# kepingbi/ProdSearch

Measured on AMD Instinct MI355X. Metric: train (u,q,i,neg) tuples/sec at bs=384, 20 neg, d=128, higher is better.
Workload: dtype f32 (fp32 MFMA and VALU; wide products, the fused per-replica kernels and grouped weight gradients as fp32-grade bf16x3 products: exact 3-way bf16 split of both fp32 operands, 6 of the 9 cross products as bf16 MFMAs per step, fp32 accumulation); 1 GPU; item_transformer d=128 1 layer 8 heads ff=512 uprev=20 bs=384/GPU 20 neg Q=8 W=1 P=18357 V=32387 dropout=0.10 (BASELINE configs[1]); global_batch=384, parallelism=dp1, step=sample+fwd+bwd+clip/Adam via nn.Module API (trainer.py:74-78), replicas_per_row=21

## Files before the change

### prodsearch_amd/csrc/rowwise.h

```cpp
#pragma once
#include "common.h"

struct ScoreArgs {
  int B, K, W, C, R, d;
  FDiv fK1, fWK1, fC;
  int64_t P, V;
  int bias_product, pos_weight;
  const int64_t* target; const int64_t* neg_items; const int64_t* pos_words; const int64_t* neg_words;
  const int64_t* candi;
  const float* product_emb; const float* word_emb; const float* product_bias; const float* word_bias;
  const float* enc;
  float* item_scores;
  float* word_scores;
  float* loss_parts;
  float* item_terms;
  float* word_terms;
  float* loss3;
  float* loss_acc;
  float* loss_blk;
  int loss_nblk;
  float scale;
  const float* scale_dev;
  float* denc;
  int part;
  int items_elsewhere;
  float* g_product_emb; float* g_word_emb; float* g_product_bias; float* g_word_bias;
  float* word_blk; int word_nblk; float* item_blk; uint32_t* ticket;
  const float* samp_prob; const int32_t* samp_alias; uint32_t samp_step, samp_k0, samp_k1; int samp_inline;
  unsigned long long* stamp;
};
#define PS_WORD_TASKS_PER_WG 16
inline void score_finish(ScoreArgs& a) {
  a.fK1 = make_fdiv(a.K + 1); a.fWK1 = make_fdiv(a.W * (a.K + 1)); a.fC = make_fdiv(a.C > 0 ? a.C : 1);
}
int launch_score_fwd(ScoreArgs& a, hipStream_t st);
int launch_loss(const ScoreArgs& a, hipStream_t st);
int launch_score_bwd(const ScoreArgs& a, hipStream_t st);

struct WSplit {
  const float* w[3]; int rows[3], cols[3];
  uint16_t* fwd_wo; uint16_t* fwd_ff; uint16_t* bwd_ff; uint16_t* bwd_wo;
  int on;
  const float* wkv[2]; uint16_t* fwd_kv;
  uint16_t* bwd_kv;
};
__host__ __device__ inline int wsplit_chunks(const WSplit& W, int ) {
  const int d = W.cols[0], F = W.rows[1];
  return (d * d + 2 * d * F) / 8 + (W.wkv[0] ? 2 * d * d / 8 : 0);
}
#if defined(__HIPCC__)
__device__ inline void wsplit_chunk(const WSplit& W, int set, int q) {
  const int d = W.cols[0], F = W.rows[1];
  const int n_wo = d * d / 8, n_ff = 2 * d * F / 8, n_kv = W.wkv[0] ? 2 * d * d / 8 : 0;
  if (q >= n_wo + n_ff + n_kv) return;
  uint16_t* dst;
  int which;
  if (q < n_wo) { which = set ? 3 : 0; dst = set ? W.bwd_wo : W.fwd_wo; }
  else if (q < n_wo + n_ff) { which = set ? 2 : 1; q -= n_wo; dst = set ? W.bwd_ff : W.fwd_ff; }
  else { which = set ? 5 : 4; q -= n_wo + n_ff; dst = set ? W.bwd_kv : W.fwd_kv; }
  const int step = q >> 6, ln = q & 63, l31 = ln & 31, hh = ln >> 5;
  const int phi = 16 * ((l31 >> 2) & 1) + 4 * (l31 >> 3) + (l31 & 3);
  const float* src; int stride;
  if (which == 0) { const int nb = step >> 3, t = step & 7; src = W.w[0] + (size_t)(32 * nb + phi) * d + 16 * t + 8 * hh; stride = 1; }
  else if (which == 4) { const int nb = step >> 3, t = step & 7; src = W.wkv[nb >> 2] + (size_t)(32 * (nb & 3) + phi) * d + 16 * t + 8 * hh; stride = 1; }
  else if (which == 5) {
    const int hg = step >> 5, nb = (step >> 3) & 3, t = step & 7;
    src = W.wkv[t >> 2] + (size_t)(64 * hg + 16 * (t & 3) + 8 * hh) * d + 32 * nb + phi; stride = d;
  }
  else if (which == 3) { const int kb = step >> 3, t = step & 7; src = W.w[0] + (size_t)(16 * t + 8 * hh) * d + 32 * kb + phi; stride = d; }
  else {
    const int fb = step >> 4, r = step & 15;
    if (r < 8) {
      if (which == 1) { src = W.w[1] + (size_t)(32 * fb + phi) * d + 16 * r + 8 * hh; stride = 1; }
      else { src = W.w[2] + (size_t)(16 * r + 8 * hh) * F + 32 * fb + phi; stride = F; }
    } else {
      const int t = (r - 8) >> 2, nb = (r - 8) & 3, kf = 32 * fb + 16 * hh + 8 * t;
      if (which == 1) { src = W.w[2] + (size_t)(32 * nb + phi) * F + kf; stride = 1; }
      else { src = W.w[1] + (size_t)kf * d + 32 * nb + phi; stride = d; }
    }
  }
  float x[8];
  if (stride == 1) {
    const float4 v0 = *reinterpret_cast<const float4*>(src), v1 = *reinterpret_cast<const float4*>(src + 4);
    x[0] = v0.x; x[1] = v0.y; x[2] = v0.z; x[3] = v0.w; x[4] = v1.x; x[5] = v1.y; x[6] = v1.z; x[7] = v1.w;
  } else {
#pragma unroll
    for (int e = 0; e < 8; ++e) x[e] = src[(size_t)e * stride];
  }
  uint32_t wd[3][4];
#pragma unroll
  for (int i = 0; i < 4; ++i) {
    uint16_t hb[2][3];
#pragma unroll
    for (int e = 0; e < 2; ++e) {
      const float xv = x[2 * i + e];
      const __bf16 bh = (__bf16)xv;
      float r = xv - (float)bh;
      const __bf16 bm = (__bf16)r;
      r -= (float)bm;
      const __bf16 bl = (__bf16)r;
      hb[e][0] = __builtin_bit_cast(uint16_t, bh); hb[e][1] = __builtin_bit_cast(uint16_t, bm); hb[e][2] = __builtin_bit_cast(uint16_t, bl);
    }
#pragma unroll
    for (int pl = 0; pl < 3; ++pl) wd[pl][i] = (uint32_t)hb[0][pl] | ((uint32_t)hb[1][pl] << 16);
  }
#pragma unroll
  for (int pl = 0; pl < 3; ++pl)
    *reinterpret_cast<uint4*>(dst + ((size_t)(step * 3 + pl) * 64 + ln) * 8) = make_uint4(wd[pl][0], wd[pl][1], wd[pl][2], wd[pl][3]);
}
#endif
struct EmbedArgs {
  int B, Q, L, S, d;
  int64_t P, V;
  int tem;
  int fs;
  const float* fs_w; const float* fs_b;
  int32_t* vrows; int32_t* vcount;
  int samp_wgs;
  int use_pos;
  const int64_t* qw; const int64_t* ui;
  const float* word_emb; const float* hist_tab; const float* pe;
  DropSpec drop_fs;
  float* qmean_d;
  float* query_emb;
  float* x;
  const float* samp_prob; const int32_t* samp_alias; int64_t* samp_items; int64_t* samp_words;
  int samp_nitem, samp_nword; uint32_t samp_step, samp_k0, samp_k1;
  int fold_words; ScoreArgs sc; int word_wgs, list_wgs;
  WSplit split; int split_wgs;
  int split_fwd_only;
  uint32_t* clear_word;
  int32_t* zero_i32; int zero_n, zero_wgs;
};
int launch_embed_fwd(const EmbedArgs& a, hipStream_t st);

struct LnFwdArgs {
  const float* x; int ldx; float* y; int ldy; float* stats;
  const float* g; const float* b; int rows, d; float eps;
};
int launch_ln_fwd(const LnFwdArgs& a, hipStream_t st);

struct LnBwdArgs {
  const float* dy; int lddy;
  const float* x; int ldx;
  const float* stats; const float* g;
  int rows, d;
  ResMap res;
  float* dx; int lddx;
  float* out2;
  DropSpec drop2;
  float* colsum;
  float* dgamma; float* dbeta;
  float* partial;
};
int launch_ln_bwd(const LnBwdArgs& a, hipStream_t st);
int ln_bwd_blocks(int rows);

#define PS_MAX_COLFOLD 8
struct ColFold { const float* partial; int nblk, d; float* dst[3]; };
struct ColFoldList { ColFold e[PS_MAX_COLFOLD]; int n; };

struct AttnArgs {
  int n_in, fan, H, S, Sq, d, dh, qpos;
  FDiv fS, fd, fdh, fd4, fHS, fHQS;
  int jc;
  int seq_div;
  int L; int64_t P; const int64_t* ui;
  const float* valid;
  const float* kp; const float* vp; const float* qp;
  float* attn;
  float* ctx;
  DropSpec drop;
  const float* dctx;
  float* dq; int lddq;
  float* dkv; int lddkv;
  float* dbq; float* dbk; float* dbv;
  float* bias_part;
  float qscale;
  const float* wq; float* dxq_part;
  const float* fanin_src;
  uint32_t* sig; uint32_t sigval;
  const uint16_t* kvb_stream; float* dxp[2];
};
inline void attn_finish(AttnArgs& a) {
  a.fS = make_fdiv(a.S); a.fd = make_fdiv(a.d); a.fdh = make_fdiv(a.dh); a.fd4 = make_fdiv(a.d / 4);
  a.fHS = make_fdiv(a.H * a.S); a.fHQS = make_fdiv((a.H / 4 > 0 ? a.H / 4 : 1) * a.S);
}
int launch_attn_fwd(const AttnArgs& a, hipStream_t st);
int launch_attn_bwd(const AttnArgs& a, hipStream_t st);
struct KvqArgs {
  AttnArgs at;
  const float* x;
  const uint16_t* kv_stream;
  const float* bk; const float* bv; const float* wq; const float* bq;
  float* kp; float* vp; float* qp;
  uint32_t* amask;
  unsigned long long* stamp;
  WSplit split;
};
bool kvq_attn_fits(const AttnArgs& a);
int launch_kvq_attn_fwd(const KvqArgs& a, hipStream_t st);
int launch_attn_fwd_sq1(const AttnArgs& a, hipStream_t st);
int launch_attn_bwd_sq1(const AttnArgs& a, hipStream_t st);
bool attn_sq1_fits(const AttnArgs& a);
bool attn_w1_fits(const AttnArgs& a);
int launch_attn_bwd_w1(const AttnArgs& a, bool pads_unread, hipStream_t st);
int launch_attn_fwd_w1(const AttnArgs& a, hipStream_t st);
bool attn_wf_fits(const AttnArgs& a);
int launch_attn_fwd_wf(const AttnArgs& a, uint32_t* amask, hipStream_t st);
int launch_attn_bwd_wf(const AttnArgs& a, const uint32_t* amask, bool pads_unread, hipStream_t st, bool* key_split = nullptr);
bool attn_bwd_wf_two_partials(const AttnArgs& a);
int attn_sq1_split(const AttnArgs& a);

struct EmbedBwdArgs {
  int B, Q, L, S, d;
  int64_t P, V;
  int tem;
  const int64_t* qw; const int64_t* ui;
  const float* dx;
  const float* dx2;
  const float* dqmean_d;
  DropSpec drop_fs;
  float* g_hist_tab; float* g_word_emb;
  const float* fw_dy; const float* fw_x; float* g_fs_w;
  const float* fsb_dqe; int fsb_lddqe; const float* fsb_qe; const float* fsb_w; float* g_fs_b;
  const float* fsb_dqe2; float fsb_k2;
  float* fsb_dqpre_out;
  ColFoldList fold;
  float* det_dm;
  uint32_t* sig; uint32_t sigval;
};
int launch_embed_scatter(const EmbedBwdArgs& a, hipStream_t st);
int launch_rows_scatter_det(const int32_t* keys, int ntask, const float* src, int64_t ld, int d, float* table, hipStream_t st,
                            const float* scale = nullptr, const int32_t* rowidx = nullptr);

int launch_fanin_sum(const float* src, int ld, int n_in, int fan, int d, float* out, hipStream_t st);
int launch_tanh_bwd(const float* dqe, int lddqe, const float* qe, float* dqpre, float* dfb, int rows, int d,
                    hipStream_t st);

struct StageArgs {
  const int64_t* src[6]; int64_t* dst[6]; int n[6];
  uint32_t step; uint32_t* step_word;
  const float* prob; const int32_t* alias;
  int nitem, nword; int64_t P, V; uint32_t k0, k1;
};
int launch_stage(const StageArgs& a, hipStream_t st);
const void* stage_kernel_handle();
const void* loss_kernel_handle();
int score_fwd_blocks(const ScoreArgs& a);

int launch_sample(const PsTemDesc& d, const float* alias_prob, const int32_t* alias_idx, int64_t* neg_items,
                  int64_t* neg_words, hipStream_t st);

struct MlpFwdArgs {
  int M, F;
  int fan, S, qpos;
  const float* ctx; const float* xin;
  const float *wo, *bo, *g1, *be1, *w1, *b1, *w2, *b2, *gf, *bef;
  DropSpec drop_ctx, drop_ff1, drop_ff2;
  float *y1, *ln1, *st1, *a1, *h1, *y2, *stf, *enc;
  int fold_score; ScoreArgs sc;
  WSplit x3;
  unsigned long long* stamp;
};
int launch_mlp_fwd_fused(const MlpFwdArgs& a, hipStream_t st);
bool mlp_fwd_can_fold_score(int M, int F, int d);
bool mlp_x3_enabled(int F);
bool mlp_fused_serves(int d, int F);
int64_t mlp_x3_floats(int d, int F);
bool ps_fusion_enabled();

struct MlpBwdArgs {
  int M, F;
  const float* denc;
  const float* item_scores; const int64_t* target; const int64_t* neg_items; const float* product_emb;
  int B, K, pos_weight; int64_t P; float scale; const float* scale_dev;
  const float* enc; float* g_product_emb; float* g_product_bias;
  const float* y2; const float* stf; const float* gf;
  const float* y1; const float* st1; const float* g1;
  const float* a1;
  const float *wo, *w1, *w2;
  DropSpec drop_ctx, drop_ff1, drop_ff2;
  float* do2;
  float* da1;
  float* dy1;
  float* dout;
  float* dctx;
  float* part_f;
  float* part_1;
  float* part_b1;
  WSplit x3;
  uint32_t* sig; uint32_t sigval;
  unsigned long long* stamp;
};
int launch_mlp_bwd_fused(const MlpBwdArgs& a, hipStream_t st);
int mlp_bwd_fused_blocks(int M);
int mlp_bwd_b1_rows(int M, int F);
```

### prodsearch_amd/csrc/rowwise.hip

```cpp
#include "rowwise.h"
#include "side_stream.h"
#include <stdlib.h>

static inline int lpr_for(int d) {
  int n = d / 4, l = 1;
  while (l < n && l < 64) l <<= 1;
  return l;
}

__device__ inline int64_t clamp_idx(int64_t i, int64_t hi) { return i < 0 ? hi : (i > hi ? hi : i); }

struct Task {
  const float* row; const float* vec; float bias; float* out;
  float* term; float tw;
  float lw;
};
__device__ inline Task score_task(const ScoreArgs& a, int t) {
  Task k;
  const int K1 = a.K + 1;
  if (a.C > 0) {
    int b = fdiv(t, a.fC);
    int64_t idx = clamp_idx(a.candi[t], a.P);
    k.row = a.product_emb + (size_t)idx * a.d;
    k.vec = a.enc + (size_t)b * a.R * a.d;
    k.bias = a.bias_product ? a.product_bias[idx] : 0.f;
    k.out = a.item_scores + t;
    k.term = nullptr; k.tw = 0.f; k.lw = 0.f;
    return k;
  }
  const int nitem = a.B * K1;
  if (t < nitem) {
    int b = fdiv(t, a.fK1), j = t - b * K1;
    int64_t idx = clamp_idx(j == 0 ? a.target[b] : a.neg_items[(size_t)b * a.K + j - 1], a.P);
    k.row = a.product_emb + (size_t)idx * a.d;
    k.vec = a.enc + ((size_t)b * a.R + (a.R > 1 ? j : 0)) * a.d;
    k.bias = a.bias_product ? a.product_bias[idx] : 0.f;
    k.out = a.item_scores + t;
    k.term = a.item_terms + t;
    k.tw = j == 0 ? -(a.pos_weight ? (float)a.K : 1.f) : 1.f;
    k.lw = 1.f;
  } else {
    int u = t - nitem;
    int b = fdiv(u, a.fWK1), r = u - b * (a.W * K1);
    int w = fdiv(r, a.fK1), j = r - w * K1;
    int64_t widx;
    if (j == 0) widx = a.pos_words[(size_t)b * a.W + w];
    else if (a.samp_inline) {
      const uint32_t su = (uint32_t)(b * a.W * a.K + w * a.K + j - 1);
      Philox4 rr = philox4x32_10(su, 0u, PS_SITE_SAMPLE_WORD, a.samp_step, a.samp_k0, a.samp_k1);
      const int64_t i = (int64_t)(((uint64_t)rr.x * (uint64_t)a.V) >> 32);
      const float f = (float)(rr.y >> 8) * (1.0f / 16777216.0f);
      widx = f < a.samp_prob[i] ? i : (int64_t)a.samp_alias[i];
    } else widx = a.neg_words[(size_t)b * a.W * a.K + (size_t)w * a.K + j - 1];
    int64_t idx = clamp_idx(widx, a.V - 1);
    int64_t tb = clamp_idx(a.target[b], a.P);
    k.row = a.word_emb + (size_t)idx * a.d;
    k.vec = a.product_emb + (size_t)tb * a.d;
    k.bias = a.word_bias[idx];
    k.out = a.word_scores + u;
    k.term = a.word_terms + u;
    k.tw = j == 0 ? -1.f : 1.f;
    int cnt = 0;
    for (int ww = 0; ww < a.W; ++ww) cnt += a.pos_words[(size_t)b * a.W + ww] != a.V - 1;
    const bool valid = a.pos_words[(size_t)b * a.W + w] != a.V - 1;
    k.lw = valid ? -1.f / (float)cnt : -0.f;
  }
  return k;
}


__device__ inline void word_tasks_wg(const ScoreArgs& a, int wg) {
  __shared__ float wred[16];
  const int tid = threadIdx.x, grp = tid >> 4, c = tid & 15;
  const int nitem = a.B * (a.K + 1), nword = a.B * a.W * (a.K + 1);
  const int nch = a.d >> 2;
  float cil = 0.f;
  if (wg == 0 && tid < 18) a.ticket[tid] = 0u;
  for (int pass = 0; pass < PS_WORD_TASKS_PER_WG / 16; ++pass) {
    const int u = wg * PS_WORD_TASKS_PER_WG + pass * 16 + grp;
    float s = 0.f;
    Task k;
    k.out = nullptr;
    if (u < nword) {
      k = score_task(a, nitem + u);
      for (int cc = c; cc < nch; cc += 16) {
        const float4 r = *reinterpret_cast<const float4*>(k.row + 4 * cc);
        const float4 v = *reinterpret_cast<const float4*>(k.vec + 4 * cc);
        s += r.x * v.x + r.y * v.y + r.z * v.z + r.w * v.w;
      }
    }
    s = group_sum(s, 16);
    if (c == 0 && k.out) {
      const float sc = s + k.bias;
      *k.out = sc;
      const float term = fabsf(k.tw) * softplus_f(k.tw < 0.f ? -sc : sc);
      *k.term = term;
      cil -= term * k.lw;
    }
  }
  if (c == 0) wred[grp] = cil;
  __syncthreads();
  if (tid == 0) {
    float q = 0.f;
    for (int g2 = 0; g2 < 16; ++g2) q += wred[g2];
    a.word_blk[wg] = q;
  }
}

__global__ __launch_bounds__(256) void embed_fwd_kernel(const EmbedArgs a) {
  extern __shared__ float red[];
  if ((int)blockIdx.x >= a.B && (int)blockIdx.x < a.B + a.samp_wgs) {
    const int t = ((int)blockIdx.x - a.B) * 256 + (int)threadIdx.x;
    if (t < a.samp_nitem) {
      Philox4 r = philox4x32_10((uint32_t)t, 0u, PS_SITE_SAMPLE_ITEM, a.samp_step, a.samp_k0, a.samp_k1);
      a.samp_items[t] = (int64_t)(((uint64_t)r.x * (uint64_t)a.P) >> 32);
    } else if (t < a.samp_nitem + a.samp_nword) {
      const int u = t - a.samp_nitem;
      Philox4 r = philox4x32_10((uint32_t)u, 0u, PS_SITE_SAMPLE_WORD, a.samp_step, a.samp_k0, a.samp_k1);
      const int64_t i = (int64_t)(((uint64_t)r.x * (uint64_t)a.V) >> 32);
      const float f = (float)(r.y >> 8) * (1.0f / 16777216.0f);
      a.samp_words[u] = f < a.samp_prob[i] ? i : (int64_t)a.samp_alias[i];
    }
    return;
  }
  if ((int)blockIdx.x >= a.B + a.samp_wgs + a.list_wgs + a.word_wgs + a.split_wgs) {
    const int i = (((int)blockIdx.x - a.B - a.samp_wgs - a.list_wgs - a.word_wgs - a.split_wgs) * 256 + (int)threadIdx.x) * 4;
    if (i + 3 < a.zero_n) *reinterpret_cast<int4*>(a.zero_i32 + i) = make_int4(0, 0, 0, 0);
    else for (int j = i; j < a.zero_n; ++j) a.zero_i32[j] = 0;
    return;
  }
  if ((int)blockIdx.x >= a.B + a.samp_wgs + a.list_wgs + a.word_wgs) {
    const int q = ((int)blockIdx.x - a.B - a.samp_wgs - a.list_wgs - a.word_wgs) * 256 + (int)threadIdx.x;
    const int n0 = wsplit_chunks(a.split, 0);
    if (q < n0) wsplit_chunk(a.split, 0, q);
    else if (!a.split_fwd_only) wsplit_chunk(a.split, 1, q - n0);
    return;
  }
  if ((int)blockIdx.x >= a.B + a.samp_wgs + a.list_wgs) {
    word_tasks_wg(a.sc, (int)blockIdx.x - a.B - a.samp_wgs - a.list_wgs);
    return;
  }
  if ((int)blockIdx.x >= a.B + a.samp_wgs) {
    __shared__ int vred[4];
    const int b = (int)blockIdx.x - a.B - a.samp_wgs, tid = threadIdx.x;
    int cntp = 0;
    {
      const int n = b * a.L;
      const bool al16 = (reinterpret_cast<uintptr_t>(a.ui) & 15) == 0;
      if (al16) {
        const longlong2* u2 = reinterpret_cast<const longlong2*>(a.ui);
        const int n2 = n >> 1;
        for (int i = tid; i < n2; i += 4 * 256) {
          longlong2 v[4];
#pragma unroll
          for (int u = 0; u < 4; ++u) { const int j = i + 256 * u; v[u] = u2[j < n2 ? j : 0]; }
#pragma unroll
          for (int u = 0; u < 4; ++u) {
            const int j = i + 256 * u;
            cntp += (j < n2 && v[u].x != a.P) + (j < n2 && v[u].y != a.P);
          }
        }
        if ((n & 1) && tid == 0) cntp += (a.ui[n - 1] != a.P);
      } else {
        for (int i = tid; i < n; i += 256) cntp += (a.ui[i] != a.P);
      }
    }
    const bool mine = tid < a.L && a.ui[(size_t)b * a.L + tid] != a.P;
    const unsigned long long vm = __ballot(mine);
    cntp = (int)wave_sum((float)cntp);
    if ((tid & 63) == 0) vred[tid >> 6] = cntp;
    __syncthreads();
    const int off = vred[0] + vred[1] + vred[2] + vred[3] + b;
    if (tid == 0) a.vrows[off] = b * a.S;
    if (mine) a.vrows[off + 1 + __popcll(vm & ((1ull << tid) - 1ull))] = b * a.S + 1 + tid;
    if (tid == 0 && b == a.B - 1) *a.vcount = off + 1 + __popcll(vm);
    return;
  }
  const int b = blockIdx.x, tid = threadIdx.x;
  if (b == 0 && tid == 0 && a.clear_word) { a.clear_word[0] = 0u; a.clear_word[1] = 0u; a.clear_word[2] = 0u; a.clear_word[3] = 0u; }
  const int d = a.d, nchunk = d >> 2;
  const int rpp = 256 / nchunk;
  const int rg = tid / nchunk, c = tid - rg * nchunk;
  const bool active = rg < rpp;
  const bool fuse_fs = a.fs && a.fs_w;
  float* mean_s = red + (size_t)rpp * d;
  const bool fs_pre = fuse_fs && d == 128;
  float4 wpre[16];
  float4 bpre = make_float4(0.f, 0.f, 0.f, 0.f);
  if (fs_pre) {
#pragma unroll
    for (int u = 0; u < 16; ++u) wpre[u] = *reinterpret_cast<const float4*>(a.fs_w + (size_t)(rg + 8 * u) * 128 + 4 * c);
  }
  if (fuse_fs && tid < nchunk) bpre = *reinterpret_cast<const float4*>(a.fs_b + 4 * c);
  const int64_t wpad = a.V - 1;
  int cnt = 0;
  for (int q = 0; q < a.Q; ++q) cnt += (a.qw[(size_t)b * a.Q + q] != wpad);
  float4 acc = make_float4(0.f, 0.f, 0.f, 0.f);
  if (active) {
    for (int q = rg; q < a.Q; q += rpp) {
      int64_t idx = a.qw[(size_t)b * a.Q + q];
      if (idx != wpad && idx >= 0 && idx < a.V) {
        float4 v = *reinterpret_cast<const float4*>(a.word_emb + (size_t)idx * d + 4 * c);
        acc.x += v.x; acc.y += v.y; acc.z += v.z; acc.w += v.w;
      }
    }
    *reinterpret_cast<float4*>(red + (size_t)rg * d + 4 * c) = acc;
  }
  __syncthreads();
  if (tid < nchunk) {
    float4 s = make_float4(0.f, 0.f, 0.f, 0.f);
    for (int r = 0; r < rpp; ++r) {
      float4 v = *reinterpret_cast<const float4*>(red + (size_t)r * d + 4 * c);
      s.x += v.x; s.y += v.y; s.z += v.z; s.w += v.w;
    }
    const float inv = 1.f / (float)(cnt > 0 ? cnt : 1);
    float m[4] = {s.x * inv, s.y * inv, s.z * inv, s.w * inv};
#pragma unroll
    for (int e = 0; e < 4; ++e) m[e] *= drop_mult(a.drop_fs, (uint32_t)b, (uint32_t)(4 * c + e));
    float4 md = make_float4(m[0], m[1], m[2], m[3]);
    *reinterpret_cast<float4*>(a.qmean_d + (size_t)b * d + 4 * c) = md;
    if (fuse_fs) *reinterpret_cast<float4*>(mean_s + 4 * c) = md;
    if (!a.fs) {
      *reinterpret_cast<float4*>(a.query_emb + (size_t)b * d + 4 * c) = md;
      if (a.tem) {
        float4 o = md;
        if (a.use_pos) {
          float4 p = *reinterpret_cast<const float4*>(a.pe + 4 * c);
          o.x += p.x; o.y += p.y; o.z += p.z; o.w += p.w;
        }
        *reinterpret_cast<float4*>(a.x + (size_t)b * a.S * d + 4 * c) = o;
      }
    }
  }
  if (a.tem && active) {
    for (int l = rg; l < a.L; l += rpp) {
      int64_t idx = a.ui[(size_t)b * a.L + l];
      float4 v = make_float4(0.f, 0.f, 0.f, 0.f);
      if (idx != a.P && idx >= 0 && idx < a.P)
        v = *reinterpret_cast<const float4*>(a.hist_tab + (size_t)idx * d + 4 * c);
      if (a.use_pos) {
        float4 p = *reinterpret_cast<const float4*>(a.pe + (size_t)(1 + l) * d + 4 * c);
        v.x += p.x; v.y += p.y; v.z += p.z; v.w += p.w;
      }
      *reinterpret_cast<float4*>(a.x + ((size_t)b * a.S + 1 + l) * d + 4 * c) = v;
    }
  }
  if (!fuse_fs) return;
  __syncthreads();
  float* out_s = mean_s + d;
  if (fs_pre) {
    const float4 mv = *reinterpret_cast<const float4*>(mean_s + 4 * c);
#pragma unroll
    for (int u = 0; u < 16; ++u) {
      const float4 wv = wpre[u];
      const float s = half_sum_last(wv.x * mv.x + wv.y * mv.y + wv.z * mv.z + wv.w * mv.w);
      if (c == 31) out_s[rg + 8 * u] = s;
    }
  } else {
    int lpr = 1;
    while (lpr < nchunk && lpr < 64) lpr <<= 1;
    const int ngrp = 256 / lpr, grp = tid / lpr, lc = tid - grp * lpr;
    for (int o0 = grp; o0 < d; o0 += 4 * ngrp) {
      float part[4];
#pragma unroll
      for (int u = 0; u < 4; ++u) {
        const int o = o0 + u * ngrp;
        float s = 0.f;
        if (o < d)
          for (int cc = lc; cc < nchunk; cc += lpr) {
            const float4 wv = *reinterpret_cast<const float4*>(a.fs_w + (size_t)o * d + 4 * cc);
            const float4 mv = *reinterpret_cast<const float4*>(mean_s + 4 * cc);
            s += wv.x * mv.x + wv.y * mv.y + wv.z * mv.z + wv.w * mv.w;
          }
        part[u] = s;
      }
#pragma unroll
      for (int u = 0; u < 4; ++u) {
        const int o = o0 + u * ngrp;
        const float s = lpr == 32 ? half_sum_last(part[u]) : group_sum(part[u], lpr);
        if (lc == lpr - 1 && o < d) out_s[o] = s;
      }
    }
  }
  __syncthreads();
  if (tid < nchunk) {
    float4 y = *reinterpret_cast<const float4*>(out_s + 4 * c);
    y.x = tanh_fast(y.x + bpre.x); y.y = tanh_fast(y.y + bpre.y); y.z = tanh_fast(y.z + bpre.z); y.w = tanh_fast(y.w + bpre.w);
    *reinterpret_cast<float4*>(a.query_emb + (size_t)b * d + 4 * c) = y;
    if (a.tem) {
      if (a.use_pos) {
        float4 p = *reinterpret_cast<const float4*>(a.pe + 4 * c);
        y.x += p.x; y.y += p.y; y.z += p.z; y.w += p.w;
      }
      *reinterpret_cast<float4*>(a.x + (size_t)b * a.S * d + 4 * c) = y;
    }
  }
}

int launch_embed_fwd(const EmbedArgs& a, hipStream_t st) {
  PS_REQUIRE(a.d % 4 == 0 && a.d <= 1024, "embed: d=%d unsupported", a.d);
  int rpp = 256 / (a.d / 4);
  const int nsamp = a.samp_prob ? ps_cdiv(a.samp_nitem + a.samp_nword, 256) : 0;
  const int nlist = (a.vrows && a.tem && a.L <= 64) ? a.B : 0;
  EmbedArgs b = a;
  b.samp_wgs = nsamp;
  b.list_wgs = nlist;
  if (!nlist) b.vrows = nullptr;
  b.word_wgs = a.fold_words ? a.sc.word_nblk : 0;
  b.split_wgs = 0;
  if (a.split.on) {
    const WSplit& W = a.split;
    PS_REQUIRE(W.w[0] && W.w[1] && W.w[2] && W.fwd_wo && W.fwd_ff && W.bwd_ff && W.bwd_wo, "embed: weight split: null pointer");
    PS_REQUIRE(W.rows[0] == 128 && W.cols[0] == 128 && W.cols[1] == 128 && W.rows[2] == 128 && W.rows[1] == W.cols[2] &&
               W.rows[1] % 256 == 0, "embed: weight split: shapes [%d,%d] [%d,%d] [%d,%d]", W.rows[0], W.cols[0], W.rows[1],
               W.cols[1], W.rows[2], W.cols[2]);
    PS_REQUIRE(!W.wkv[0] || (W.wkv[1] && W.fwd_kv), "embed: weight split: K / V weights without their stream");
    PS_REQUIRE(!W.wkv[0] || W.bwd_kv, "embed: weight split: K / V weights without their backward stream");
    b.split_wgs = ps_cdiv(wsplit_chunks(W, 0) + (a.split_fwd_only ? 0 : wsplit_chunks(W, 1)), 256);
  }
  PS_REQUIRE(!a.fold_words || (a.sc.word_blk && a.sc.ticket && a.sc.d <= 512), "embed: folded word tasks need their buffers");
  b.zero_wgs = a.zero_i32 && a.zero_n > 0 ? ps_cdiv(a.zero_n, 1024) : 0;
  PS_REQUIRE(!b.zero_wgs || ((uintptr_t)a.zero_i32 & 15) == 0, "embed: zero_i32 must be 16-byte aligned");
  hipLaunchKernelGGL(embed_fwd_kernel, dim3(a.B + nsamp + nlist + b.word_wgs + b.split_wgs + b.zero_wgs), dim3(256),
                     (size_t)(rpp + 2) * a.d * sizeof(float), st, b);
  PS_LAUNCH_CHECK();
  return PS_OK;
}

#define LN_MAXI 8
template <int DPL>
__global__ __launch_bounds__(256) void ln_fwd_kernel(const LnFwdArgs a) {
  const int lane = threadIdx.x & 63;
  const int wave = (blockIdx.x * blockDim.x + threadIdx.x) >> 6;
  const int nw = (gridDim.x * blockDim.x) >> 6;
  const float invd = 1.f / (float)a.d;
  for (int row = wave; row < a.rows; row += nw) {
    float v[DPL];
    float s = 0.f;
#pragma unroll
    for (int i = 0; i < DPL; ++i) {
      int col = lane + 64 * i;
      v[i] = col < a.d ? a.x[(size_t)row * a.ldx + col] : 0.f;
      s += v[i];
    }
    const float mean = wave_sum(s) * invd;
    float q = 0.f;
#pragma unroll
    for (int i = 0; i < DPL; ++i) {
      int col = lane + 64 * i;
      float t = col < a.d ? v[i] - mean : 0.f;
      q += t * t;
    }
    const float rstd = 1.f / sqrtf(wave_sum(q) * invd + a.eps);
#pragma unroll
    for (int i = 0; i < DPL; ++i) {
      int col = lane + 64 * i;
      if (col < a.d) a.y[(size_t)row * a.ldy + col] = (v[i] - mean) * rstd * a.g[col] + a.b[col];
    }
    if (lane == 0) { a.stats[2 * (size_t)row] = mean; a.stats[2 * (size_t)row + 1] = rstd; }
  }
}

int launch_ln_fwd(const LnFwdArgs& a, hipStream_t st) {
  PS_REQUIRE(a.d <= 64 * LN_MAXI, "layernorm: d=%d > %d", a.d, 64 * LN_MAXI);
  int blocks = ps_cdiv(a.rows, 4);
  if (blocks > 4096) blocks = 4096;
  const int dpl = ps_cdiv(a.d, 64);
  if (dpl <= 1) hipLaunchKernelGGL(ln_fwd_kernel<1>, dim3(blocks), dim3(256), 0, st, a);
  else if (dpl <= 2) hipLaunchKernelGGL(ln_fwd_kernel<2>, dim3(blocks), dim3(256), 0, st, a);
  else if (dpl <= 4) hipLaunchKernelGGL(ln_fwd_kernel<4>, dim3(blocks), dim3(256), 0, st, a);
  else hipLaunchKernelGGL(ln_fwd_kernel<8>, dim3(blocks), dim3(256), 0, st, a);
  PS_LAUNCH_CHECK();
  return PS_OK;
}

#define LNB_WAVES 16
template <int DPL, int EXACT>
__global__ __launch_bounds__(64 * LNB_WAVES) void ln_bwd_kernel(const LnBwdArgs a) {
  extern __shared__ float sh[];
  const int W = 64 * DPL;
  const int lane = threadIdx.x & 63, wv = threadIdx.x >> 6;
  const int wave = (blockIdx.x * blockDim.x + threadIdx.x) >> 6;
  const int nw = (gridDim.x * blockDim.x) >> 6;
  const float invd = 1.f / (float)a.d;
  float ag[DPL], ab[DPL], ac[DPL];
#pragma unroll
  for (int i = 0; i < DPL; ++i) { ag[i] = 0.f; ab[i] = 0.f; ac[i] = 0.f; }
  if (EXACT) {
    float gv[DPL];
#pragma unroll
    for (int i = 0; i < DPL; ++i) gv[i] = a.g[lane + 64 * i];
    const int rmode = a.res.mode;
    DropSpec d2 = a.drop2;
    d2.step = drop_step(a.drop2); d2.step_ptr = nullptr;
    for (int row = wave; row < a.rows; row += nw) {
      const float mean = a.stats[2 * (size_t)row], rstd = a.stats[2 * (size_t)row + 1];
      float xv[DPL], dyv[DPL], rres[DPL];
#pragma unroll
      for (int i = 0; i < DPL; ++i) {
        xv[i] = a.x[(size_t)row * a.ldx + lane + 64 * i];
        dyv[i] = a.dy[(size_t)row * a.lddy + lane + 64 * i];
        rres[i] = 0.f;
      }
      if (rmode == RES_DIRECT) {
#pragma unroll
        for (int i = 0; i < DPL; ++i) rres[i] = a.res.ptr[(size_t)row * a.res.ld + lane + 64 * i];
      } else if (rmode != RES_NONE) {
#pragma unroll
        for (int i = 0; i < DPL; ++i) rres[i] = res_value(a.res, row, lane + 64 * i);
      }
      float xh[DPL], dxh[DPL];
      float s1 = 0.f, s2 = 0.f;
#pragma unroll
      for (int i = 0; i < DPL; ++i) {
        xh[i] = (xv[i] - mean) * rstd;
        dxh[i] = dyv[i] * gv[i];
        s1 += dxh[i];
        s2 += dxh[i] * xh[i];
      }
      s1 = wave_sum(s1) * invd;
      s2 = wave_sum(s2) * invd;
      float dx[DPL];
#pragma unroll
      for (int i = 0; i < DPL; ++i) {
        dx[i] = rstd * (dxh[i] - s1 - xh[i] * s2);
        if (rmode != RES_NONE) dx[i] += rres[i];
        a.dx[(size_t)row * a.lddx + lane + 64 * i] = dx[i];
        ag[i] += dyv[i] * xh[i];
        ab[i] += dyv[i];
      }
      if (a.out2) {
#pragma unroll
        for (int i = 0; i < DPL; ++i) {
          const float v2 = dx[i] * drop_mult(d2, (uint32_t)row, (uint32_t)(lane + 64 * i));
          a.out2[(size_t)row * a.d + lane + 64 * i] = v2;
          ac[i] += v2;
        }
      } else {
#pragma unroll
        for (int i = 0; i < DPL; ++i) ac[i] += dx[i];
      }
    }
  } else
  for (int row = wave; row < a.rows; row += nw) {
    const float mean = a.stats[2 * (size_t)row], rstd = a.stats[2 * (size_t)row + 1];
    float xh[DPL], dxh[DPL], dyv[DPL];
    float s1 = 0.f, s2 = 0.f;
#pragma unroll
    for (int i = 0; i < DPL; ++i) {
      int col = lane + 64 * i;
      if (col < a.d) {
        float x = a.x[(size_t)row * a.ldx + col];
        dyv[i] = a.dy[(size_t)row * a.lddy + col];
        xh[i] = (x - mean) * rstd;
        dxh[i] = dyv[i] * a.g[col];
      } else { xh[i] = 0.f; dxh[i] = 0.f; dyv[i] = 0.f; }
      s1 += dxh[i];
      s2 += dxh[i] * xh[i];
    }
    s1 = wave_sum(s1) * invd;
    s2 = wave_sum(s2) * invd;
#pragma unroll
    for (int i = 0; i < DPL; ++i) {
      int col = lane + 64 * i;
      if (col < a.d) {
        float dx = rstd * (dxh[i] - s1 - xh[i] * s2);
        if (a.res.mode != RES_NONE) dx += res_value(a.res, row, col);
        a.dx[(size_t)row * a.lddx + col] = dx;
        float v2 = dx;
        if (a.out2) {
          v2 = dx * drop_mult(a.drop2, (uint32_t)row, (uint32_t)col);
          a.out2[(size_t)row * a.d + col] = v2;
        }
        ag[i] += dyv[i] * xh[i];
        ab[i] += dyv[i];
        ac[i] += v2;
      }
    }
  }
#pragma unroll
  for (int i = 0; i < DPL; ++i) {
    sh[(0 * LNB_WAVES + wv) * W + lane + 64 * i] = ag[i];
    sh[(1 * LNB_WAVES + wv) * W + lane + 64 * i] = ab[i];
    sh[(2 * LNB_WAVES + wv) * W + lane + 64 * i] = ac[i];
  }
  __syncthreads();
  for (int t = threadIdx.x; t < 3 * a.d; t += blockDim.x) {
    const int which = t / a.d, col = t - which * a.d;
    float* dst = which == 0 ? a.dgamma : (which == 1 ? a.dbeta : a.colsum);
    if (!dst && !a.partial) continue;
    float s = 0.f;
    for (int w = 0; w < LNB_WAVES; ++w) s += sh[(which * LNB_WAVES + w) * W + col];
    if (a.partial) a.partial[((size_t)blockIdx.x * 3 + which) * a.d + col] = s;
    else atomicAdd(&dst[col], s);
  }
}

__global__ __launch_bounds__(64 * LNB_WAVES) void ln_bwd_v4_kernel(const LnBwdArgs a) {
  extern __shared__ float sh[];
  const int lane = threadIdx.x & 63, wv = threadIdx.x >> 6;
  const int wave = (blockIdx.x * blockDim.x + threadIdx.x) >> 6;
  const int nw = (gridDim.x * blockDim.x) >> 6;
  const float invd = 1.f / 256.f;
  const float4 gv = reinterpret_cast<const float4*>(a.g)[lane];
  const bool has_res = a.res.mode == RES_DIRECT;
  DropSpec d2 = a.drop2;
  d2.step = drop_step(a.drop2); d2.step_ptr = nullptr;
  float4 ag = make_float4(0.f, 0.f, 0.f, 0.f), ab = ag, ac = ag;
  for (int row0 = wave; row0 < a.rows; row0 += 2 * nw) {
    const bool two = row0 + nw < a.rows;
    const int rw[2] = {row0, two ? row0 + nw : row0};
    float4 xv[2], dyv[2], rr[2];
    float2 st[2];
#pragma unroll
    for (int u = 0; u < 2; ++u) {
      st[u] = reinterpret_cast<const float2*>(a.stats)[rw[u]];
      xv[u] = *reinterpret_cast<const float4*>(a.x + (size_t)rw[u] * a.ldx + 4 * lane);
      dyv[u] = *reinterpret_cast<const float4*>(a.dy + (size_t)rw[u] * a.lddy + 4 * lane);
      rr[u] = has_res ? *reinterpret_cast<const float4*>(a.res.ptr + (size_t)rw[u] * a.res.ld + 4 * lane) : make_float4(0.f, 0.f, 0.f, 0.f);
    }
#pragma unroll
    for (int u = 0; u < 2; ++u) {
      if (u == 1 && !two) break;
      const float mean = st[u].x, rstd = st[u].y;
      const float xh[4] = {(xv[u].x - mean) * rstd, (xv[u].y - mean) * rstd, (xv[u].z - mean) * rstd, (xv[u].w - mean) * rstd};
      const float dy[4] = {dyv[u].x, dyv[u].y, dyv[u].z, dyv[u].w};
      const float g4[4] = {gv.x, gv.y, gv.z, gv.w};
      const float r4[4] = {rr[u].x, rr[u].y, rr[u].z, rr[u].w};
      float dxh[4], s1 = 0.f, s2 = 0.f;
#pragma unroll
      for (int i = 0; i < 4; ++i) { dxh[i] = dy[i] * g4[i]; s1 += dxh[i]; s2 += dxh[i] * xh[i]; }
      s1 = wave_sum(s1) * invd;
      s2 = wave_sum(s2) * invd;
      float dx[4];
#pragma unroll
      for (int i = 0; i < 4; ++i) dx[i] = rstd * (dxh[i] - s1 - xh[i] * s2) + r4[i];
      *reinterpret_cast<float4*>(a.dx + (size_t)rw[u] * a.lddx + 4 * lane) = make_float4(dx[0], dx[1], dx[2], dx[3]);
      ag.x += dy[0] * xh[0]; ag.y += dy[1] * xh[1]; ag.z += dy[2] * xh[2]; ag.w += dy[3] * xh[3];
      ab.x += dy[0]; ab.y += dy[1]; ab.z += dy[2]; ab.w += dy[3];
      if (a.out2) {
        float v2[4];
#pragma unroll
        for (int i = 0; i < 4; ++i) v2[i] = dx[i] * drop_mult(d2, (uint32_t)rw[u], (uint32_t)(4 * lane + i));
        *reinterpret_cast<float4*>(a.out2 + (size_t)rw[u] * 256 + 4 * lane) = make_float4(v2[0], v2[1], v2[2], v2[3]);
        ac.x += v2[0]; ac.y += v2[1]; ac.z += v2[2]; ac.w += v2[3];
      } else {
        ac.x += dx[0]; ac.y += dx[1]; ac.z += dx[2]; ac.w += dx[3];
      }
    }
  }
  *reinterpret_cast<float4*>(sh + (0 * LNB_WAVES + wv) * 256 + 4 * lane) = ag;
  *reinterpret_cast<float4*>(sh + (1 * LNB_WAVES + wv) * 256 + 4 * lane) = ab;
  *reinterpret_cast<float4*>(sh + (2 * LNB_WAVES + wv) * 256 + 4 * lane) = ac;
  __syncthreads();
  for (int t = threadIdx.x; t < 3 * 256; t += blockDim.x) {
    const int which = t >> 8, col = t & 255;
    float* dst = which == 0 ? a.dgamma : (which == 1 ? a.dbeta : a.colsum);
    if (!dst && !a.partial) continue;
    float s = 0.f;
    for (int w = 0; w < LNB_WAVES; ++w) s += sh[(which * LNB_WAVES + w) * 256 + col];
    if (a.partial) a.partial[((size_t)blockIdx.x * 3 + which) * 256 + col] = s;
    else atomicAdd(&dst[col], s);
  }
}
static bool ln_bwd_v4_takes(const LnBwdArgs& a) {
  if (a.d != 256 || (a.res.mode != RES_NONE && a.res.mode != RES_DIRECT)) return false;
  uintptr_t bits = (uintptr_t)a.x | (uintptr_t)a.dy | (uintptr_t)a.dx | (uintptr_t)a.g | (uintptr_t)a.out2 | (uintptr_t)a.stats;
  int lds = a.ldx | a.lddy | a.lddx;
  if (a.res.mode == RES_DIRECT) { bits |= (uintptr_t)a.res.ptr; lds |= a.res.ld; }
  return (bits & 15) == 0 && (lds & 3) == 0;
}

int ln_bwd_blocks(int rows) {
  int blocks = ps_cdiv(rows, LNB_WAVES);
  return blocks > 256 ? 256 : blocks;
}

int launch_ln_bwd(const LnBwdArgs& a, hipStream_t st) {
  PS_REQUIRE(a.d <= 64 * LN_MAXI, "layernorm bwd: d=%d > %d", a.d, 64 * LN_MAXI);
  const int blocks = ln_bwd_blocks(a.rows);
  const int dpl = ps_cdiv(a.d, 64);
  const int dp = dpl <= 1 ? 1 : (dpl <= 2 ? 2 : (dpl <= 4 ? 4 : 8));
  const size_t lds = sizeof(float) * 3 * LNB_WAVES * 64 * dp;
  const dim3 blk(64 * LNB_WAVES);
  const bool exact = a.d == 64 * dp;
  if (ln_bwd_v4_takes(a)) {
    hipLaunchKernelGGL(ln_bwd_v4_kernel, dim3(blocks), blk, sizeof(float) * 3 * LNB_WAVES * 256, st, a);
    PS_LAUNCH_CHECK();
    return PS_OK;
  }
#define LNB_LAUNCH(DP_)                                                                           \
  do {                                                                                            \
    if (exact) hipLaunchKernelGGL((ln_bwd_kernel<DP_, 1>), dim3(blocks), blk, lds, st, a);         \
    else hipLaunchKernelGGL((ln_bwd_kernel<DP_, 0>), dim3(blocks), blk, lds, st, a);               \
  } while (0)
  if (dp == 1) LNB_LAUNCH(1);
  else if (dp == 2) LNB_LAUNCH(2);
  else if (dp == 4) LNB_LAUNCH(4);
  else LNB_LAUNCH(8);
#undef LNB_LAUNCH
  PS_LAUNCH_CHECK();
  return PS_OK;
}

struct AttnLds {
  float *Ks, *Vs, *Qs, *Ps, *Pd, *valid;
};
__device__ inline AttnLds attn_carve(float* base, int S, int Sq, int dh) {
  AttnLds l;
  l.Ks = base; base += S * dh;
  l.Vs = base; base += S * dh;
  l.Qs = base; base += Sq * dh;
  l.Ps = base; base += Sq * (S + 1);
  l.Pd = base; base += Sq * (S + 1);
  l.valid = base;
  return l;
}
static inline size_t attn_fwd_lds(int S, int Sq, int dh) {
  return sizeof(float) * ((size_t)2 * S * dh + Sq * dh + 2 * Sq * (S + 1) + S);
}

__device__ inline void attn_load_common(const AttnArgs& a, const AttnLds& l, int b, int h, int tid) {
  const int S = a.S, Sq = a.Sq, dh = a.dh, d = a.d;
  for (int i = tid; i < S * dh; i += 64) {
    int s = i / dh, c = i - s * dh;
// ... 1369 lines not shown
```

Baseline: 37.59 million tuples/s.

## Restructure embed forward to issue query, history and dropout loads up front

Reorganises the per-row embedding forward kernel so that query-word ids, history ids, history rows, positional encodings and dropout multipliers are all loaded at the start, before the first barrier. This overlaps their latency instead of running dependent gathers serially. The padding count now uses a wave ballot, and the fused projection in the d=128 path reads the mean from registers, which removes one barrier. History stores for the first slots are deferred to the end. Optional timestamp instrumentation is added behind a diagnostic flag. The cost is higher register pressure from the preloaded values.

Result: no change. 37.48 million tuples/s (-0.3%).

```diff
diff --git a/prodsearch_amd/csrc/rowwise.h b/prodsearch_amd/csrc/rowwise.h
--- a/prodsearch_amd/csrc/rowwise.h
+++ b/prodsearch_amd/csrc/rowwise.h
@@ -131,7 +131,11 @@
   int split_fwd_only;
   uint32_t* clear_word;
   int32_t* zero_i32; int zero_n, zero_wgs;
-};
+  unsigned long long* stamp;
+};
+#define PS_EMB_UQ 1
+#define PS_EMB_UH 3
+__host__ __device__ inline int embed_slot(int first, int rg, int rpp, int u) { return first + rg + rpp * u; }
 int launch_embed_fwd(const EmbedArgs& a, hipStream_t st);
 
 struct LnFwdArgs {
diff --git a/prodsearch_amd/csrc/rowwise.hip b/prodsearch_amd/csrc/rowwise.hip
--- a/prodsearch_amd/csrc/rowwise.hip
+++ b/prodsearch_amd/csrc/rowwise.hip
@@ -50,7 +50,9 @@
       Philox4 rr = philox4x32_10(su, 0u, PS_SITE_SAMPLE_WORD, a.samp_step, a.samp_k0, a.samp_k1);
       const int64_t i = (int64_t)(((uint64_t)rr.x * (uint64_t)a.V) >> 32);
       const float f = (float)(rr.y >> 8) * (1.0f / 16777216.0f);
-      widx = f < a.samp_prob[i] ? i : (int64_t)a.samp_alias[i];
+      const float pr = a.samp_prob[i];
+      const int32_t al = a.samp_alias[i];
+      widx = f < pr ? i : (int64_t)al;
     } else widx = a.neg_words[(size_t)b * a.W * a.K + (size_t)w * a.K + j - 1];
     int64_t idx = clamp_idx(widx, a.V - 1);
     int64_t tb = clamp_idx(a.target[b], a.P);
@@ -107,8 +109,25 @@
   }
 }
 
+#if PS_DIAG_ON
+#define EMB_STAMP(slot)                                                                                  \
+  do {                                                                                                   \
+    if (a.stamp && threadIdx.x == 0) {                                                                   \
+      unsigned long long t_;                                                                             \
+      asm volatile("s_memrealtime %0\n\ts_waitcnt lgkmcnt(0)" : "=s"(t_)::"memory");                    \
+      a.stamp[16 * (size_t)blockIdx.x + (slot)] = t_;                                                    \
+    }                                                                                                    \
+  } while (0)
+#define EMB_WAIT() do { if (a.stamp) asm volatile("s_waitcnt vmcnt(0)" ::: "memory"); } while (0)
+#define EMB_END(kind) do { EMB_STAMP(7); if (a.stamp && threadIdx.x == 0) a.stamp[16 * (size_t)blockIdx.x + 8] = (kind) + 1; } while (0)
+#else
+#define EMB_STAMP(slot) do { } while (0)
+#define EMB_WAIT() do { } while (0)
+#define EMB_END(kind) do { } while (0)
+#endif
 __global__ __launch_bounds__(256) void embed_fwd_kernel(const EmbedArgs a) {
   extern __shared__ float red[];
+  EMB_STAMP(0);
   if ((int)blockIdx.x >= a.B && (int)blockIdx.x < a.B + a.samp_wgs) {
     const int t = ((int)blockIdx.x - a.B) * 256 + (int)threadIdx.x;
     if (t < a.samp_nitem) {
@@ -119,14 +138,18 @@
       Philox4 r = philox4x32_10((uint32_t)u, 0u, PS_SITE_SAMPLE_WORD, a.samp_step, a.samp_k0, a.samp_k1);
       const int64_t i = (int64_t)(((uint64_t)r.x * (uint64_t)a.V) >> 32);
       const float f = (float)(r.y >> 8) * (1.0f / 16777216.0f);
-      a.samp_words[u] = f < a.samp_prob[i] ? i : (int64_t)a.samp_alias[i];
-    }
+      const float pr = a.samp_prob[i];
+      const int32_t al = a.samp_alias[i];
+      a.samp_words[u] = f < pr ? i : (int64_t)al;
+    }
+    EMB_END(1);
     return;
   }
   if ((int)blockIdx.x >= a.B + a.samp_wgs + a.list_wgs + a.word_wgs + a.split_wgs) {
     const int i = (((int)blockIdx.x - a.B - a.samp_wgs - a.list_wgs - a.word_wgs - a.split_wgs) * 256 + (int)threadIdx.x) * 4;
     if (i + 3 < a.zero_n) *reinterpret_cast<int4*>(a.zero_i32 + i) = make_int4(0, 0, 0, 0);
     else for (int j = i; j < a.zero_n; ++j) a.zero_i32[j] = 0;
+    EMB_END(5);
     return;
   }
   if ((int)blockIdx.x >= a.B + a.samp_wgs + a.list_wgs + a.word_wgs) {
@@ -134,10 +157,12 @@
     const int n0 = wsplit_chunks(a.split, 0);
     if (q < n0) wsplit_chunk(a.split, 0, q);
     else if (!a.split_fwd_only) wsplit_chunk(a.split, 1, q - n0);
+    EMB_END(4);
     return;
   }
   if ((int)blockIdx.x >= a.B + a.samp_wgs + a.list_wgs) {
     word_tasks_wg(a.sc, (int)blockIdx.x - a.B - a.samp_wgs - a.list_wgs);
+    EMB_END(3);
     return;
   }
   if ((int)blockIdx.x >= a.B + a.samp_wgs) {
@@ -174,6 +199,7 @@
     if (tid == 0) a.vrows[off] = b * a.S;
     if (mine) a.vrows[off + 1 + __popcll(vm & ((1ull << tid) - 1ull))] = b * a.S + 1 + tid;
     if (tid == 0 && b == a.B - 1) *a.vcount = off + 1 + __popcll(vm);
+    EMB_END(2);
     return;
   }
   const int b = blockIdx.x, tid = threadIdx.x;
@@ -183,73 +209,158 @@
   const int rg = tid / nchunk, c = tid - rg * nchunk;
   const bool active = rg < rpp;
   const bool fuse_fs = a.fs && a.fs_w;
+  const bool hist = a.tem && a.L > 0, pos = a.tem && a.use_pos;
   float* mean_s = red + (size_t)rpp * d;
+  const int64_t* __restrict__ qrow = a.qw + (size_t)b * a.Q;
+  const int64_t* __restrict__ urow = a.ui + (size_t)b * a.L;
+  const float* __restrict__ wtab = a.word_emb + 4 * c;
+  const float* __restrict__ htab = a.hist_tab + 4 * c;
+  const float* __restrict__ pe = a.pe + 4 * c;
+  float* __restrict__ xrow = a.x + (size_t)b * a.S * d + 4 * c;
+  float* __restrict__ qmean_d = a.qmean_d + (size_t)b * d + 4 * c;
+  float* __restrict__ query_emb = a.query_emb + (size_t)b * d + 4 * c;
   const bool fs_pre = fuse_fs && d == 128;
+  DropSpec dfs = a.drop_fs;
+  if (dfs.step_ptr) dfs.step = *reinterpret_cast<const volatile uint32_t*>(dfs.step_ptr);
+  dfs.step_ptr = nullptr;
   float4 wpre[16];
-  float4 bpre = make_float4(0.f, 0.f, 0.f, 0.f);
+  float4 bpre = make_float4(0.f, 0.f, 0.f, 0.f), p0 = bpre;
   if (fs_pre) {
 #pragma unroll
     for (int u = 0; u < 16; ++u) wpre[u] = *reinterpret_cast<const float4*>(a.fs_w + (size_t)(rg + 8 * u) * 128 + 4 * c);
   }
-  if (fuse_fs && tid < nchunk) bpre = *reinterpret_cast<const float4*>(a.fs_b + 4 * c);
   const int64_t wpad = a.V - 1;
-  int cnt = 0;
-  for (int q = 0; q < a.Q; ++q) cnt += (a.qw[(size_t)b * a.Q + q] != wpad);
+  int64_t qid[PS_EMB_UQ], hid[PS_EMB_UH], cid = wpad;
+  float4 hp[PS_EMB_UH];
+  if (a.Q > 0) {
+#pragma unroll
+    for (int u = 0; u < PS_EMB_UQ; ++u) qid[u] = qrow[min(embed_slot(0, rg, rpp, u), a.Q - 1)];
+    cid = qrow[min(tid & 63, a.Q - 1)];
+  }
+  if (hist) {
+#pragma unroll
+    for (int u = 0; u < PS_EMB_UH; ++u) hid[u] = urow[min(embed_slot(0, rg, rpp, u), a.L - 1)];
+  }
+  if (fuse_fs) bpre = *reinterpret_cast<const float4*>(a.fs_b + 4 * c);
+  if (pos) p0 = *reinterpret_cast<const float4*>(pe);
+  const bool means = tid < nchunk || fs_pre;
+  float dm[4] = {1.f, 1.f, 1.f, 1.f};
+  if (means) {
+#pragma unroll
+    for (int e = 0; e < 4; ++e) dm[e] = drop_mult(dfs, (uint32_t)b, (uint32_t)(4 * c + e));
+  }
+  asm volatile("" : "+v"(cid), "+v"(p0.x), "+v"(bpre.x));
+#if PS_DIAG_ON
+  if (a.stamp) { asm volatile("" ::"v"(qid[0]), "v"(hid[0])); asm volatile("s_waitcnt vmcnt(0)" ::: "memory"); }
+#endif
+  EMB_STAMP(1);
+  int cnt = __popcll(__ballot((tid & 63) < a.Q && cid != wpad));
+  for (int q0 = 64; q0 < a.Q; q0 += 64) {
+    const int q = q0 + (tid & 63);
+    cnt += __popcll(__ballot(q < a.Q && qrow[min(q, a.Q - 1)] != wpad));
+  }
+  float4 qv[PS_EMB_UQ], hv[PS_EMB_UH];
+  bool qon[PS_EMB_UQ], hon[PS_EMB_UH];
+  if (hist) {
+#pragma unroll
+    for (int u = 0; u < PS_EMB_UH; ++u) {
+      hon[u] = hid[u] >= 0 && hid[u] < a.P;
+      hv[u] = *reinterpret_cast<const float4*>(htab + (size_t)(hon[u] ? hid[u] : a.P) * d);
+    }
+    if (pos) {
+#pragma unroll
+      for (int u = 0; u < PS_EMB_UH; ++u) hp[u] = *reinterpret_cast<const float4*>(pe + (size_t)(1 + min(embed_slot(0, rg, rpp, u), a.L - 1)) * d);
+    }
+  }
+  if (a.Q > 0) {
+#pragma unroll
+    for (int u = 0; u < PS_EMB_UQ; ++u) {
+      qon[u] = active && embed_slot(0, rg, rpp, u) < a.Q && qid[u] >= 0 && qid[u] < wpad;
+      qv[u] = *reinterpret_cast<const float4*>(wtab + (size_t)(qon[u] ? qid[u] : wpad) * d);
+    }
+  }
   float4 acc = make_float4(0.f, 0.f, 0.f, 0.f);
-  if (active) {
-    for (int q = rg; q < a.Q; q += rpp) {
-      int64_t idx = a.qw[(size_t)b * a.Q + q];
-      if (idx != wpad && idx >= 0 && idx < a.V) {
-        float4 v = *reinterpret_cast<const float4*>(a.word_emb + (size_t)idx * d + 4 * c);
-        acc.x += v.x; acc.y += v.y; acc.z += v.z; acc.w += v.w;
-      }
-    }
-    *reinterpret_cast<float4*>(red + (size_t)rg * d + 4 * c) = acc;
-  }
+  if (a.Q > 0) {
+#pragma unroll
+    for (int u = 0; u < PS_EMB_UQ; ++u) {
+      acc.x += qon[u] ? qv[u].x : 0.f; acc.y += qon[u] ? qv[u].y : 0.f; acc.z += qon[u] ? qv[u].z : 0.f; acc.w += qon[u] ? qv[u].w : 0.f;
+    }
+  }
+  for (int q0 = rpp * PS_EMB_UQ; q0 < a.Q; q0 += rpp * PS_EMB_UQ) {
+#pragma unroll
+    for (int u = 0; u < PS_EMB_UQ; ++u) qid[u] = qrow[min(embed_slot(q0, rg, rpp, u), a.Q - 1)];
+#pragma unroll
+    for (int u = 0; u < PS_EMB_UQ; ++u) {
+      qon[u] = active && embed_slot(q0, rg, rpp, u) < a.Q && qid[u] >= 0 && qid[u] < wpad;
+      qv[u] = *reinterpret_cast<const float4*>(wtab + (size_t)(qon[u] ? qid[u] : wpad) * d);
+    }
+#pragma unroll
+    for (int u = 0; u < PS_EMB_UQ; ++u) {
+      acc.x += qon[u] ? qv[u].x : 0.f; acc.y += qon[u] ? qv[u].y : 0.f; acc.z += qon[u] ? qv[u].z : 0.f; acc.w += qon[u] ? qv[u].w : 0.f;
+    }
+  }
+#if PS_DIAG_ON
+  if (a.stamp) { asm volatile("" ::"v"(acc.x), "v"(hv[0].x)); asm volatile("s_waitcnt vmcnt(0)" ::: "memory"); }
+#endif
+  EMB_STAMP(2);
+  if (active) *reinterpret_cast<float4*>(red + (size_t)rg * d + 4 * c) = acc;
+  if (hist) {
+#pragma unroll
+    for (int u = 0; u < PS_EMB_UH; ++u) {
+      hv[u] = make_float4(hon[u] ? hv[u].x : 0.f, hon[u] ? hv[u].y : 0.f, hon[u] ? hv[u].z : 0.f, hon[u] ? hv[u].w : 0.f);
+      if (pos) { hv[u].x += hp[u].x; hv[u].y += hp[u].y; hv[u].z += hp[u].z; hv[u].w += hp[u].w; }
+      asm volatile("" : "+v"(hv[u].x), "+v"(hv[u].y), "+v"(hv[u].z), "+v"(hv[u].w));
+    }
+    for (int l = rpp * PS_EMB_UH + rg; l < a.L; l += rpp) {
+      const int64_t id = urow[l];
+      const bool on = id >= 0 && id < a.P;
+      float4 v = *reinterpret_cast<const float4*>(htab + (size_t)(on ? id : a.P) * d);
+      float4 p = make_float4(0.f, 0.f, 0.f, 0.f);
+      if (pos) p = *reinterpret_cast<const float4*>(pe + (size_t)(1 + l) * d);
+      v = make_float4(on ? v.x : 0.f, on ? v.y : 0.f, on ? v.z : 0.f, on ? v.w : 0.f);
+      if (pos) { v.x += p.x; v.y += p.y; v.z += p.z; v.w += p.w; }
+      if (active) *reinterpret_cast<float4*>(xrow + (size_t)(1 + l) * d) = v;
+    }
+  }
+  EMB_STAMP(5);
+  auto store_hist = [&]() {
+    if (!hist) return;
+#pragma unroll
+    for (int u = 0; u < PS_EMB_UH; ++u) {
+      const int l = embed_slot(0, rg, rpp, u);
+      if (active && l < a.L) *reinterpret_cast<float4*>(xrow + (size_t)(1 + l) * d) = hv[u];
+    }
+  };
   __syncthreads();
-  if (tid < nchunk) {
+  EMB_STAMP(3);
+  float4 md = make_float4(0.f, 0.f, 0.f, 0.f);
+  if (means) {
     float4 s = make_float4(0.f, 0.f, 0.f, 0.f);
+#pragma unroll 4
     for (int r = 0; r < rpp; ++r) {
       float4 v = *reinterpret_cast<const float4*>(red + (size_t)r * d + 4 * c);
       s.x += v.x; s.y += v.y; s.z += v.z; s.w += v.w;
     }
     const float inv = 1.f / (float)(cnt > 0 ? cnt : 1);
-    float m[4] = {s.x * inv, s.y * inv, s.z * inv, s.w * inv};
-#pragma unroll
-    for (int e = 0; e < 4; ++e) m[e] *= drop_mult(a.drop_fs, (uint32_t)b, (uint32_t)(4 * c + e));
-    float4 md = make_float4(m[0], m[1], m[2], m[3]);
-    *reinterpret_cast<float4*>(a.qmean_d + (size_t)b * d + 4 * c) = md;
-    if (fuse_fs) *reinterpret_cast<float4*>(mean_s + 4 * c) = md;
+    md = make_float4(s.x * inv * dm[0], s.y * inv * dm[1], s.z * inv * dm[2], s.w * inv * dm[3]);
+  }
+  if (tid < nchunk) {
+    *reinterpret_cast<float4*>(qmean_d) = md;
+    if (fuse_fs && !fs_pre) *reinterpret_cast<float4*>(mean_s + 4 * c) = md;
     if (!a.fs) {
-      *reinterpret_cast<float4*>(a.query_emb + (size_t)b * d + 4 * c) = md;
+      *reinterpret_cast<float4*>(query_emb) = md;
       if (a.tem) {
         float4 o = md;
-        if (a.use_pos) {
-          float4 p = *reinterpret_cast<const float4*>(a.pe + 4 * c);
-          o.x += p.x; o.y += p.y; o.z += p.z; o.w += p.w;
-        }
-        *reinterpret_cast<float4*>(a.x + (size_t)b * a.S * d + 4 * c) = o;
-      }
-    }
-  }
-  if (a.tem && active) {
-    for (int l = rg; l < a.L; l += rpp) {
-      int64_t idx = a.ui[(size_t)b * a.L + l];
-      float4 v = make_float4(0.f, 0.f, 0.f, 0.f);
-      if (idx != a.P && idx >= 0 && idx < a.P)
-        v = *reinterpret_cast<const float4*>(a.hist_tab + (size_t)idx * d + 4 * c);
-      if (a.use_pos) {
-        float4 p = *reinterpret_cast<const float4*>(a.pe + (size_t)(1 + l) * d + 4 * c);
-        v.x += p.x; v.y += p.y; v.z += p.z; v.w += p.w;
-      }
-      *reinterpret_cast<float4*>(a.x + ((size_t)b * a.S + 1 + l) * d + 4 * c) = v;
-    }
-  }
-  if (!fuse_fs) return;
-  __syncthreads();
+        if (pos) { o.x += p0.x; o.y += p0.y; o.z += p0.z; o.w += p0.w; }
+        *reinterpret_cast<float4*>(xrow) = o;
+      }
+    }
+  }
+  EMB_STAMP(4);
+  if (!fuse_fs) { store_hist(); EMB_END(0); return; }
   float* out_s = mean_s + d;
   if (fs_pre) {
-    const float4 mv = *reinterpret_cast<const float4*>(mean_s + 4 * c);
+    const float4 mv = md;
 #pragma unroll
     for (int u = 0; u < 16; ++u) {
       const float4 wv = wpre[u];
@@ -257,6 +368,7 @@
       if (c == 31) out_s[rg + 8 * u] = s;
     }
   } else {
+    __syncthreads();
     int lpr = 1;
     while (lpr < nchunk && lpr < 64) lpr <<= 1;
     const int ngrp = 256 / lpr, grp = tid / lpr, lc = tid - grp * lpr;
@@ -283,18 +395,18 @@
     }
   }
   __syncthreads();
+  EMB_STAMP(6);
   if (tid < nchunk) {
     float4 y = *reinterpret_cast<const float4*>(out_s + 4 * c);
     y.x = tanh_fast(y.x + bpre.x); y.y = tanh_fast(y.y + bpre.y); y.z = tanh_fast(y.z + bpre.z); y.w = tanh_fast(y.w + bpre.w);
-    *reinterpret_cast<float4*>(a.query_emb + (size_t)b * d + 4 * c) = y;
+    *reinterpret_cast<float4*>(query_emb) = y;
     if (a.tem) {
-      if (a.use_pos) {
-        float4 p = *reinterpret_cast<const float4*>(a.pe + 4 * c);
-        y.x += p.x; y.y += p.y; y.z += p.z; y.w += p.w;
-      }
-      *reinterpret_cast<float4*>(a.x + (size_t)b * a.S * d + 4 * c) = y;
-    }
-  }
+      if (pos) { y.x += p0.x; y.y += p0.y; y.z += p0.z; y.w += p0.w; }
+      *reinterpret_cast<float4*>(xrow) = y;
+    }
+  }
+  store_hist();
+  EMB_END(0);
 }
 
 int launch_embed_fwd(const EmbedArgs& a, hipStream_t st) {
@@ -321,6 +433,9 @@
   PS_REQUIRE(!a.fold_words || (a.sc.word_blk && a.sc.ticket && a.sc.d <= 512), "embed: folded word tasks need their buffers");
   b.zero_wgs = a.zero_i32 && a.zero_n > 0 ? ps_cdiv(a.zero_n, 1024) : 0;
   PS_REQUIRE(!b.zero_wgs || ((uintptr_t)a.zero_i32 & 15) == 0, "embed: zero_i32 must be 16-byte aligned");
+#if PS_DIAG_ON
+  b.stamp = (ps_diag_int("PS_EMB_STAMP", 0) && a.B + nsamp + nlist + b.word_wgs + b.split_wgs + b.zero_wgs <= 4096) ? ps_debug_stamp_ptr() : nullptr;
+#endif
   hipLaunchKernelGGL(embed_fwd_kernel, dim3(a.B + nsamp + nlist + b.word_wgs + b.split_wgs + b.zero_wgs), dim3(256),
                      (size_t)(rpp + 2) * a.d * sizeof(float), st, b);
   PS_LAUNCH_CHECK();
```
